# vocdoni/zk-franchise-proof-circuit

Measured on AMD Instinct MI355X. Metric: zkCensus proofs/sec (nLevels=160), higher is better.
Workload: dtype u256 (8 x u32 Montgomery, BN254 Fr/Fq)

## Files before the change

### include/zkcensus.h

```cpp
#ifndef ZKCENSUS_H
#define ZKCENSUS_H
#include <stddef.h>
#include <stdint.h>
#ifdef __cplusplus
extern "C" {
#endif

typedef struct zkc_ctx zkc_ctx;
typedef struct zkc_zkey zkc_zkey;

enum {
    ZKC_OK = 0,
    ZKC_ERR_GENERIC = 1,
    ZKC_ERR_SHORT_BUFFER = 2,
    ZKC_ERR_INVALID_WITNESS_LENGTH = 3,
    ZKC_ERR_BAD_ARG = 4,
    ZKC_ERR_FORMAT = 5,
    ZKC_ERR_HIP = 6,
    ZKC_ERR_WITNESS = 7
};
enum {
    ZKC_W_OK = 0, ZKC_W_ERR_WEIGHT = 1 , ZKC_W_ERR_SIK_ROOT = 2 ,
    ZKC_W_ERR_CENSUS_ROOT = 3 , ZKC_W_ERR_NULLIFIER = 4 , ZKC_W_ERR_LAST_SIBLING = 5 ,
    ZKC_W_ERR_INPUT_RANGE = 6 ,
// ... 81 lines not shown

int zkc_verify_batch(zkc_ctx* ctx, const uint8_t* vk, int nPublic, const uint8_t* pubs, const uint8_t* proofs, int N, const uint8_t* seed32);
const char* zkc_verify_last_error(void);

int zkc_proof_to_json(const uint8_t proof[256], const uint8_t* pub, int nPublic, char* proof_buf, unsigned long* proof_size,
                      char* public_buf, unsigned long* public_size);
int zkc_proof_from_json(const char* proof_json, const char* public_json, uint8_t proof[256], uint8_t* pub, int* nPublic);
int zkc_vkey_from_json(const char* vkey_json, uint8_t* vk, unsigned long* vk_size, int* nPublic);
int zkc_wtns_parse(const void* wtns_bytes, unsigned long size, const uint8_t** payload, uint32_t* nWitness);
unsigned long zkc_wtns_write(const void* payload, uint32_t nWitness, void* out, unsigned long out_size);

typedef struct zkc_msm zkc_msm;
int zkc_ntt_dev(zkc_ctx* ctx, const void* d_src, void* d_dst, int logn, int nvec, int inverse);
int zkc_g1_mul_batch_dev(zkc_ctx* ctx, const uint8_t base_std[64], const void* d_scalars, uint32_t n, void* d_out);
int zkc_msm_g1_load_dev(zkc_ctx* ctx, const void* d_bases_std, uint32_t n, zkc_msm** out);
int zkc_msm_g1_dev(zkc_msm* m, const void* d_scalars, uint8_t out[64]);
void zkc_msm_g1_free(zkc_msm* m);

int zkc_debug_stage(zkc_zkey* zk, const void* d_wtns, int stage, void* host_out);
unsigned long long zkc_debug_early_retries(void);
int zkc_msm_debug(zkc_zkey* zk, int which, const void* d_scalars, uint32_t count, void* host_out);
int zkc_debug_pairing_dev(zkc_ctx* ctx, const uint8_t* g1, const uint8_t* g2, const uint8_t* weights, int N, uint8_t product_out[384], uint8_t* folded_out,
                          int32_t* member_out, int* bad_out, const uint32_t* nodes, size_t count, uint8_t* node_out);

int zkc_poseidon_batch(zkc_ctx* ctx, int n_inputs, const void* inputs, size_t B, void* out);
int zkc_smt_build(zkc_ctx* ctx, const void* keys, const void* values, size_t n, int nLevels, uint8_t root[32], void* siblings, int32_t* depths);
int zkc_census_inputs(zkc_ctx* ctx, size_t n, int nLevels, const uint8_t election_id[64], const void* address, const void* password, const void* signature,
                      const void* available_weight, const void* vote_weight, const void* vote_hash, void* inputs_out, void* d_inputs_out, uint8_t* roots_out);

typedef struct zkc_tree zkc_tree;
enum {
    ZKC_TREE_OK = 0,
    ZKC_TREE_KEY_EXISTS = 1,
    ZKC_TREE_KEY_ABSENT = 2,
    ZKC_TREE_COLLISION = 3,
    ZKC_TREE_NOT_BELOW_R = 4,
    ZKC_TREE_NOT_IN_CENSUS = 5,
    ZKC_TREE_NOT_IN_SIK = 6,
    ZKC_TREE_SIK_MISMATCH = 7
};
int  zkc_tree_create(zkc_ctx* ctx, int nLevels, zkc_tree** out);
void zkc_tree_free(zkc_tree* tree);
int  zkc_tree_add(zkc_tree* tree, const void* keys, const void* values, size_t n, int32_t* status);
int  zkc_tree_update(zkc_tree* tree, const void* keys, const void* values, size_t n, int32_t* status);
int  zkc_tree_root(zkc_tree* tree, uint8_t root[32]);
int  zkc_tree_size(zkc_tree* tree, size_t* leaves);
// ... 38 lines not shown
```

### zk-franchise-proof-circuit_amd/__init__.py

```python
import ctypes
from . import _native
from ._native import ZkcError
from .inputs import INPUT_KEYS, flatten_inputs, R_MOD

__all__ = ['Context', 'ProvingKey', 'DevicePool', 'ProvingService', 'groth16', 'ZkcError', 'INPUT_KEYS', 'flatten_inputs', 'R_MOD']


class Context:

    def __init__(self, device=0):
        self._lib = _native.load()
        h = ctypes.c_void_p()
        rc = self._lib.zkc_ctx_create(int(device), ctypes.byref(h))
        if rc != 0:
            raise ZkcError(rc, (self._lib.zkc_last_error(None) or b'').decode())
        self._h = h
        self.device = device
        self._keys = []

    def close(self):
        if getattr(self, '_h', None):
            for k in list(self._keys):
                k.close()
            self._lib.zkc_ctx_destroy(self._h)
# ... 12 lines not shown

    @property
    def stream(self):
        return self._lib.zkc_ctx_stream(self._h)

    def n_wires(self, nLevels=160):
        return self._lib.zkc_circuit_n_wires(nLevels)

    def n_inputs(self, nLevels=160):
        return self._lib.zkc_circuit_n_inputs(nLevels)

    def witness(self, inputs, nLevels=160):
        flat = b''.join(x if isinstance(x, (bytes, bytearray)) else flatten_inputs(x, nLevels) for x in inputs)
        B = len(inputs)
        nw = self.n_wires(nLevels)
        out = ctypes.create_string_buffer(B * nw * 32)
        st = (ctypes.c_int32 * B)()
        self._check(self._lib.zkc_witness(self._h, nLevels, flat, B, out, st), allow=(7,))
        raw = out.raw
        return [raw[i * nw * 32:(i + 1) * nw * 32] for i in range(B)], list(st)

    def witness_dev(self, d_inputs_ptr, B, d_wtns_ptr, d_status_ptr, nLevels=160):
        self._check(self._lib.zkc_witness_dev(self._h, nLevels, d_inputs_ptr, B, d_wtns_ptr, d_status_ptr))


class ProvingKey:

    def __init__(self, ctx, zkey_bytes):
        self.ctx = ctx
        self._lib = ctx._lib
        h = ctypes.c_void_p()
        ctx._check(self._lib.zkc_zkey_load(ctx._h, zkey_bytes, len(zkey_bytes), ctypes.byref(h)))
        self._h = h
        ctx._keys.append(self)
        a, b, c = ctypes.c_uint32(), ctypes.c_uint32(), ctypes.c_uint32()
        self._lib.zkc_zkey_info(h, ctypes.byref(a), ctypes.byref(b), ctypes.byref(c))
        self.n_vars, self.n_public, self.domain_size = a.value, b.value, c.value
        ps, ln = ctypes.c_int(), ctypes.c_int()
        self._lib.zkc_zkey_pass_info(h, ctypes.byref(ps), ctypes.byref(ln))
        self.pass_size, self.lanes = ps.value, ln.value

    def close(self):
        if getattr(self, '_h', None):
            if getattr(self.ctx, '_h', None):
                self._lib.zkc_zkey_free(self._h)
            self._h = None
# ... 161 lines not shown
```

### zk-franchise-proof-circuit_amd/_native.py

```python
import ctypes
import os

_HERE = os.path.dirname(os.path.abspath(__file__))
LIB_PATH = os.environ.get('ZKCENSUS_LIB') or os.path.join(_HERE, 'libzkcensus.so')
_lib = None


class ZkcError(RuntimeError):
    def __init__(self, code, msg):
        super().__init__('libzkcensus error %d: %s' % (code, msg))
        self.code = code


def load():
    global _lib
    if _lib is not None:
        return _lib
    if not os.path.exists(LIB_PATH):
        raise ImportError('libzkcensus.so is not built (run `python -c "import __graft_entry__ as g; g.build()"`); '
                          'there is no CPU fallback for the product path')
    try:
        import torch
    except ImportError:
        pass
    L = ctypes.CDLL(LIB_PATH)
    vp, i32p = ctypes.c_void_p, ctypes.POINTER(ctypes.c_int32)
    L.zkc_ctx_create.argtypes = [ctypes.c_int, ctypes.POINTER(vp)]
    L.zkc_ctx_destroy.argtypes = [vp]
    L.zkc_last_error.argtypes = [vp]; L.zkc_last_error.restype = ctypes.c_char_p
    L.zkc_ctx_stream.argtypes = [vp]; L.zkc_ctx_stream.restype = vp
    L.zkc_witness.argtypes = [vp, ctypes.c_int, vp, ctypes.c_int, vp, i32p]
    L.zkc_witness_dev.argtypes = [vp, ctypes.c_int, vp, ctypes.c_int, vp, vp]
    u8p, u32p = ctypes.c_char_p, ctypes.POINTER(ctypes.c_uint32)
    L.zkc_zkey_load.argtypes = [vp, ctypes.c_char_p, ctypes.c_size_t, ctypes.POINTER(vp)]
    L.zkc_zkey_free.argtypes = [vp]; L.zkc_zkey_free.restype = None
    L.zkc_zkey_info.argtypes = [vp, u32p, u32p, u32p]
    L.zkc_zkey_pass_info.argtypes = [vp, ctypes.POINTER(ctypes.c_int), ctypes.POINTER(ctypes.c_int)]
    L.zkc_witness_status_text.argtypes = [ctypes.c_int, ctypes.c_int32]; L.zkc_witness_status_text.restype = ctypes.c_char_p
    L.zkc_prove.argtypes = [vp, ctypes.c_char_p, ctypes.c_uint32, u8p, u8p, ctypes.c_char_p, ctypes.c_char_p]
    L.zkc_prove_dev.argtypes = [vp, vp, ctypes.c_uint32, u8p, u8p, ctypes.c_char_p, ctypes.c_char_p]
    L.zkc_prove_batch_dev.argtypes = [vp, vp, ctypes.c_uint32, ctypes.c_int, ctypes.c_char_p, ctypes.c_char_p, ctypes.c_char_p]
    L.zkc_fullprove_batch_dev.argtypes = [vp, vp, ctypes.c_int, vp, vp, ctypes.c_char_p, ctypes.c_char_p, ctypes.c_char_p]
    L.zkc_debug_stage.argtypes = [vp, vp, ctypes.c_int, ctypes.c_char_p]
    L.zkc_debug_early_retries.argtypes = []; L.zkc_debug_early_retries.restype = ctypes.c_ulonglong
    L.zkc_msm_debug.argtypes = [vp, ctypes.c_int, vp, ctypes.c_uint32, ctypes.c_char_p]
    L.zkc_debug_pairing_dev.argtypes = [vp, ctypes.c_char_p, ctypes.c_char_p, ctypes.c_char_p, ctypes.c_int, ctypes.c_char_p, ctypes.c_char_p, i32p, ctypes.POINTER(ctypes.c_int),
                                        ctypes.POINTER(ctypes.c_uint32), ctypes.c_size_t, ctypes.c_char_p]
    ulp = ctypes.POINTER(ctypes.c_ulong)
    L.groth16_prover.argtypes = [ctypes.c_char_p, ctypes.c_ulong, ctypes.c_char_p, ctypes.c_ulong, ctypes.c_char_p, ulp, ctypes.c_char_p, ulp, ctypes.c_char_p, ctypes.c_ulong]
    L.zkc_verify.argtypes = [ctypes.c_char_p, ctypes.c_char_p, ctypes.c_char_p]
    L.zkc_verify_bin.argtypes = [ctypes.c_char_p, ctypes.c_int, ctypes.c_char_p, ctypes.c_char_p]
    L.zkc_verify_batch.argtypes = [vp, ctypes.c_char_p, ctypes.c_int, ctypes.c_char_p, ctypes.c_char_p, ctypes.c_int, ctypes.c_char_p]
    L.zkc_verify_batch_each.argtypes = [vp, ctypes.c_char_p, ctypes.c_int, ctypes.c_char_p, ctypes.c_char_p, ctypes.c_int, ctypes.c_char_p, i32p]
    L.zkc_verify_each_stats.argtypes = [vp, ctypes.POINTER(ctypes.c_uint64)]
    L.zkc_verify_last_error.restype = ctypes.c_char_p
    L.zkc_proof_to_json.argtypes = [ctypes.c_char_p, ctypes.c_char_p, ctypes.c_int, ctypes.c_char_p, ulp, ctypes.c_char_p, ulp]
    L.zkc_proof_from_json.argtypes = [ctypes.c_char_p, ctypes.c_char_p, ctypes.c_char_p, ctypes.c_char_p, ctypes.POINTER(ctypes.c_int)]
    L.zkc_vkey_from_json.argtypes = [ctypes.c_char_p, ctypes.c_char_p, ulp, ctypes.POINTER(ctypes.c_int)]
    L.zkc_wtns_parse.argtypes = [ctypes.c_char_p, ctypes.c_ulong, ctypes.POINTER(ctypes.c_void_p), ctypes.POINTER(ctypes.c_uint32)]
    L.zkc_wtns_write.argtypes = [ctypes.c_char_p, ctypes.c_uint32, ctypes.c_char_p, ctypes.c_ulong]; L.zkc_wtns_write.restype = ctypes.c_ulong
    L.zkc_poseidon_batch.argtypes = [vp, ctypes.c_int, ctypes.c_char_p, ctypes.c_size_t, ctypes.c_char_p]
    L.zkc_smt_build.argtypes = [vp, ctypes.c_char_p, ctypes.c_char_p, ctypes.c_size_t, ctypes.c_int, ctypes.c_char_p, ctypes.c_char_p, i32p]
    L.zkc_census_inputs.argtypes = [vp, ctypes.c_size_t, ctypes.c_int, ctypes.c_char_p, ctypes.c_char_p, ctypes.c_char_p, ctypes.c_char_p, ctypes.c_char_p, ctypes.c_char_p, ctypes.c_char_p, vp, vp, ctypes.c_char_p]
    sz = ctypes.c_size_t
    L.zkc_tree_create.argtypes = [vp, ctypes.c_int, ctypes.POINTER(vp)]
    L.zkc_tree_free.argtypes = [vp]; L.zkc_tree_free.restype = None
    L.zkc_tree_add.argtypes = [vp, ctypes.c_char_p, ctypes.c_char_p, sz, i32p]
    L.zkc_tree_update.argtypes = [vp, ctypes.c_char_p, ctypes.c_char_p, sz, i32p]
    L.zkc_tree_delete.argtypes = [vp, ctypes.c_char_p, sz, i32p]
    L.zkc_tree_refs.argtypes = [vp, ctypes.POINTER(sz)]
# ... 96 lines not shown
```

### zk-franchise-proof-circuit_amd/csrc/zkc_msm.hip

```cpp
#include <cstdio>
#include <cstddef>
#include <ctime>
#include <cstdlib>
#include <cstring>
#include <string.h>
#include <vector>
#include "zkc_prover.h"
#include "zkc_f29.h"
#include "zkc_f29_g1.h"
#include "zkc_f29_g2.h"
#include "zkc_point_ops.h"

namespace zkc {

template <class F> struct PointIO;
template <class PP> struct PointIO<Fp<PP>> {
    typedef Fp<PP> Fq;
    static __device__ __forceinline__ Affine<Fq> load(const Affine<Fq>* p) {
        const uint4* d = reinterpret_cast<const uint4*>(p); uint4 a = d[0], b = d[1], c = d[2], e = d[3];
        Affine<Fq> r;
        r.x.v[0] = a.x; r.x.v[1] = a.y; r.x.v[2] = a.z; r.x.v[3] = a.w; r.x.v[4] = b.x; r.x.v[5] = b.y; r.x.v[6] = b.z; r.x.v[7] = b.w;
        r.y.v[0] = c.x; r.y.v[1] = c.y; r.y.v[2] = c.z; r.y.v[3] = c.w; r.y.v[4] = e.x; r.y.v[5] = e.y; r.y.v[6] = e.z; r.y.v[7] = e.w;
        return r;
    }
// ... 497 lines not shown
    return fold_group_sums<Fq>(ctx, tbl, s, w, nw, sh, gs, ng, o, pt_mod, st);
}
int fold_group_sums_g1_ws(zkc_ctx* ctx, const G1Affine* tbl, const uint32_t* s, const uint32_t* w, uint32_t nw, const uint32_t* gs, uint32_t ng, G1XYZZ* d_tmp, G1XYZZ* d_out, G1XYZZ* h_out) {
    return fold_group_sums_ws<Fq>(ctx, tbl, s, w, nw, 0, gs, ng, d_tmp, d_out, h_out, 0u, ctx->stream);
}
int fold_group_sums_g2(zkc_ctx* ctx, const G2Affine* tbl, const uint32_t* s, const uint32_t* w, uint32_t nw, int32_t sh, const uint32_t* gs, uint32_t ng, G2XYZZ* o, uint32_t pt_mod, hipStream_t st) {
    return fold_group_sums<Fq2>(ctx, tbl, s, w, nw, sh, gs, ng, o, pt_mod, st);
}

static int msm_work_alloc_impl(zkc_ctx* ctx, MsmWork& w, size_t max_entries, size_t max_buckets, int max_jobs, bool g2) {
    w.max_entries = max_entries; w.max_jobs = max_jobs; w.max_buckets = max_buckets; w.xyzz_size = g2 ? sizeof(G2XYZZ) : sizeof(G1XYZZ);
    const size_t nb = max_buckets;
    w.max_segments = std::max<size_t>(max_entries / MSM_SEG + 1, (size_t)32 * 8192) + nb + 64;
    w.max_bins = (size_t)max_jobs << MSM_MAX_HBITS;
    ZKC_HIP_CHECK(ctx, hipMalloc((void**)&w.vals, max_entries * 4 + 16)); ZKC_HIP_CHECK(ctx, hipMalloc((void**)&w.vals2, max_entries * 4 + 16));
    ZKC_HIP_CHECK(ctx, hipMalloc((void**)&w.hist, w.max_bins * 4)); ZKC_HIP_CHECK(ctx, hipMalloc((void**)&w.bin_start, w.max_bins * 4));
    w.max_tilecnt = max_entries / 8 + ((size_t)max_jobs << MSM_MAX_HBITS);
    ZKC_HIP_CHECK(ctx, hipMalloc((void**)&w.tilecnt, w.max_tilecnt * 4));
    ZKC_HIP_CHECK(ctx, hipMalloc((void**)&w.off, (nb + 2) * 4)); ZKC_HIP_CHECK(ctx, hipMalloc((void**)&w.bcnt, (nb + 2) * 4)); ZKC_HIP_CHECK(ctx, hipMalloc((void**)&w.segcnt, (nb + 2) * 4));
    ZKC_HIP_CHECK(ctx, hipMalloc((void**)&w.segoff, (nb + 2) * 4)); ZKC_HIP_CHECK(ctx, hipMalloc((void**)&w.seg2bucket, w.max_segments * 4));
    ZKC_HIP_CHECK(ctx, hipMalloc((void**)&w.seglen, w.max_segments * 4)); ZKC_HIP_CHECK(ctx, hipMalloc((void**)&w.perm, w.max_segments * 4));
    w.max_lencnt = (size_t)(MSM_SEG + 1) * (w.max_segments / 256 + 2);
    ZKC_HIP_CHECK(ctx, hipMalloc((void**)&w.lencnt, w.max_lencnt * 4));
    ZKC_HIP_CHECK(ctx, hipMalloc((void**)&w.scan_blk, (std::max(nb + 2, w.max_lencnt) / 1024 + 2) * 4));
    ZKC_HIP_CHECK(ctx, hipMalloc((void**)&w.heavy, (MSM_MAX_HEAVY + 1) * 4));
    ZKC_HIP_CHECK(ctx, hipMalloc((void**)&w.d_jobs, sizeof(MsmJobList)));
    ZKC_HIP_CHECK(ctx, hipMalloc(&w.partial, w.max_segments * w.xyzz_size));
    const size_t max_vw = max_buckets / MSM_VW_MIN + (size_t)max_jobs;
    ZKC_HIP_CHECK(ctx, hipMalloc(&w.wres, 2 * max_vw * w.xyzz_size));
    ZKC_HIP_CHECK(ctx, hipMalloc((void**)&w.d_windows, max_vw * sizeof(MsmWindow))); w.max_windows = max_vw;
    w.max_tiles = max_entries / (8 * MSM_TILE_SCALARS) + (size_t)max_jobs + 1;
    ZKC_HIP_CHECK(ctx, hipMalloc((void**)&w.d_tilejob, w.max_tiles * 2));
    for (int s = 0; s < 2; s++) {
        ZKC_HIP_CHECK(ctx, hipHostMalloc((void**)&w.h_tilejob[s], w.max_tiles * 2));
        ZKC_HIP_CHECK(ctx, hipHostMalloc((void**)&w.h_jobs[s], sizeof(MsmJobList))); ZKC_HIP_CHECK(ctx, hipHostMalloc((void**)&w.h_windows[s], max_vw * sizeof(MsmWindow)));
        ZKC_HIP_CHECK(ctx, hipEventCreateWithFlags(&w.h_ev[s], hipEventDisableTiming));
    }
    ZKC_HIP_CHECK(ctx, hipMalloc(&w.results, 2 * (size_t)max_jobs * w.xyzz_size));
    ZKC_HIP_CHECK(ctx, hipHostMalloc(&w.h_results, (size_t)max_jobs * w.xyzz_size));
    return ZKC_OK;
}
int msm_work_alloc(zkc_ctx* ctx, MsmWork& w, size_t max_entries, size_t max_buckets, int max_jobs, bool g2) {
    const int rc = msm_work_alloc_impl(ctx, w, max_entries, max_buckets, max_jobs, g2);
    if (rc != ZKC_OK) msm_work_free(w);
    return rc;
}
void msm_work_free(MsmWork& w) {
// ... 142 lines not shown
```

### zk-franchise-proof-circuit_amd/csrc/zkc_msm_sort.hip

```cpp
#include "zkc_prover.h"
#include <algorithm>

namespace zkc {

struct TileState { uint32_t s[MSM_TILE_SCALARS / MSM_TILE][8]; uint32_t pt[MSM_TILE_SCALARS / MSM_TILE]; uint32_t carry[MSM_TILE_SCALARS / MSM_TILE]; bool live[MSM_TILE_SCALARS / MSM_TILE]; };
__device__ __forceinline__ void msm_tile_load(TileState& t, const MsmJob& job, uint32_t i0) {
#pragma unroll
    for (int k = 0; k < MSM_TILE_SCALARS / MSM_TILE; k++) {
        const uint32_t i = i0 + k * MSM_TILE;
        t.live[k] = i < job.count; t.pt[k] = 0; t.carry[k] = 0;
#pragma unroll
        for (int q = 0; q < 8; q++) t.s[k][q] = 0;
        if (t.live[k]) {
            const uint32_t wire = job.vmap ? job.vmap[i] : i;
            const uint4* sp = reinterpret_cast<const uint4*>(job.scalars + 8 * (size_t)wire); const uint4 a = sp[0], b = sp[1];
            t.s[k][0] = a.x; t.s[k][1] = a.y; t.s[k][2] = a.z; t.s[k][3] = a.w; t.s[k][4] = b.x; t.s[k][5] = b.y; t.s[k][6] = b.z; t.s[k][7] = b.w;
            t.pt[k] = (uint32_t)((int32_t)wire - job.pt_shift);
        }
    }
}
__device__ __forceinline__ uint32_t msm_tile_digit(TileState& t, int k, uint32_t w, uint32_t c, uint32_t& neg) {
    const uint32_t half = 1u << (c - 1), mask = (1u << c) - 1;
    const uint32_t bit = w * c, li = bit >> 5, sh = bit & 31;
    uint32_t lo = 0, hi = 0;
// ... 248 lines not shown
    if (valid && wave > 0) rank += wcnt[(wave - 1) * LEN_KEYS + key];
    return rank;
}
__global__ void __launch_bounds__(256)
zkc_msm_lenhist(const uint32_t* __restrict__ seglen, const uint32_t* __restrict__ segoff, uint32_t nbuckets, uint32_t* __restrict__ lencnt, uint32_t max_segments) {
    __shared__ uint32_t wcnt[4 * LEN_KEYS];
    uint32_t nseg = segoff[nbuckets]; if (nseg > max_segments) nseg = max_segments;
    const uint32_t s = blockIdx.x * 256 + threadIdx.x;
    const bool valid = s < nseg;
    const uint32_t key = valid ? (uint32_t)MSM_SEG - seglen[s] : ~0u;
    (void)stable_rank_256(key, valid, wcnt);
    for (uint32_t k = threadIdx.x; k < LEN_KEYS; k += 256) lencnt[(size_t)k * gridDim.x + blockIdx.x] = wcnt[3 * LEN_KEYS + k];
}
__global__ void __launch_bounds__(256)
zkc_msm_lenscatter(const uint32_t* __restrict__ seglen, const uint32_t* __restrict__ segoff, uint32_t nbuckets, const uint32_t* __restrict__ lencnt,
                   uint32_t* __restrict__ perm, uint32_t max_segments) {
    __shared__ uint32_t wcnt[4 * LEN_KEYS];
    uint32_t nseg = segoff[nbuckets]; if (nseg > max_segments) nseg = max_segments;
    const uint32_t s = blockIdx.x * 256 + threadIdx.x;
    const bool valid = s < nseg;
    const uint32_t key = valid ? (uint32_t)MSM_SEG - seglen[s] : ~0u;
    const uint32_t rank = stable_rank_256(key, valid, wcnt);
    if (valid) perm[lencnt[(size_t)key * gridDim.x + blockIdx.x] + rank] = s;
}

#define ZKC_SORT_LAUNCH_CHECK(name) do { hipError_t _e = hipGetLastError(); if (_e != hipSuccess) return zkc_fail(ctx, ZKC_ERR_HIP, std::string(name ": ") + hipGetErrorString(_e)); } while (0)

int msm_bucket_entries(zkc_ctx* ctx, MsmWork& w, const MsmJobList& jl, hipStream_t st, unsigned long long* d_entry_counter) {
    if (jl.total_bins > w.max_bins) return zkc_fail(ctx, ZKC_ERR_BAD_ARG, "msm_bucket_entries: too many level-1 bins for the work space");
    const MsmJobList* dj = (const MsmJobList*)w.d_jobs;
    if (jl.total_tilecnt > w.max_tilecnt) return zkc_fail(ctx, ZKC_ERR_BAD_ARG, "msm_bucket_entries: too many (bin, tile) counters for the work space");
    hipLaunchKernelGGL(zkc_msm_count, dim3(jl.total_tiles), dim3(MSM_TILE), 0, st, dj, (const uint16_t*)w.d_tilejob, w.tilecnt);
    ZKC_SORT_LAUNCH_CHECK("zkc_msm_count");
    hipLaunchKernelGGL(zkc_msm_binscan, dim3(jl.njobs), dim3(256), 0, st, dj, w.tilecnt, w.hist, w.bin_start, d_entry_counter);
    ZKC_SORT_LAUNCH_CHECK("zkc_msm_binscan");
    hipLaunchKernelGGL(zkc_msm_split, dim3(jl.total_tiles), dim3(MSM_TILE), 0, st, dj, (const uint16_t*)w.d_tilejob, w.tilecnt, w.vals);
    ZKC_SORT_LAUNCH_CHECK("zkc_msm_split");
    uint64_t biggest_bin = 0;
    for (int j = 0; j < jl.njobs; j++) biggest_bin = std::max<uint64_t>(biggest_bin, ((uint64_t)jl.job[j].count * jl.job[j].nw) >> jl.job[j].hbits);
    if (biggest_bin > 8192) hipLaunchKernelGGL(HIP_KERNEL_NAME(zkc_msm_bucket<true>), dim3(jl.total_bins), dim3(256), 0, st, dj, w.hist, w.bin_start, w.vals, w.vals2, w.off, w.bcnt);
    else hipLaunchKernelGGL(HIP_KERNEL_NAME(zkc_msm_bucket<false>), dim3(jl.total_bins), dim3(256), 0, st, dj, w.hist, w.bin_start, w.vals, w.vals2, w.off, w.bcnt);
    ZKC_SORT_LAUNCH_CHECK("zkc_msm_bucket");
    return ZKC_OK;
}

static int device_scan(zkc_ctx* ctx, const uint32_t* in, uint32_t* out, uint32_t* blk, uint32_t n, hipStream_t st) {
    const uint32_t nblk = (n + SCAN_PER_BLOCK - 1) / SCAN_PER_BLOCK;
    hipLaunchKernelGGL(zkc_scan_local, dim3(nblk), dim3(256), 0, st, in, out, blk, n);
    hipLaunchKernelGGL(zkc_scan_blocks, dim3(1), dim3(256), 0, st, blk, nblk);
    hipLaunchKernelGGL(zkc_scan_fix, dim3((n + 255) / 256), dim3(256), 0, st, out, blk, n);
    ZKC_SORT_LAUNCH_CHECK("zkc_scan");
    return ZKC_OK;
}
int msm_build_segments(zkc_ctx* ctx, MsmWork& w, const MsmJobList& jl, uint32_t seg, size_t seg_bound, hipStream_t st) {
    const uint32_t nb = jl.total_buckets;
    if (seg > (uint32_t)MSM_SEG) return zkc_fail(ctx, ZKC_ERR_BAD_ARG, "msm_build_segments: segment length");
    ZKC_HIP_CHECK(ctx, hipMemsetAsync(w.heavy + MSM_MAX_HEAVY, 0, 4, st));
    hipLaunchKernelGGL(zkc_msm_segcount, dim3((nb + 1 + 255) / 256), dim3(256), 0, st, w.bcnt, nb, w.segcnt, w.heavy, w.heavy + MSM_MAX_HEAVY, seg);
    ZKC_SORT_LAUNCH_CHECK("zkc_msm_segcount");
    int rc = device_scan(ctx, w.segcnt, w.segoff, w.scan_blk, nb + 1, st); if (rc) return rc;
    const bool sort_by_len = seg > (uint32_t)MSM_SEG_MIN * 2;
    hipLaunchKernelGGL(zkc_msm_seg2bucket, dim3((nb + 255) / 256), dim3(256), 0, st, w.bcnt, w.segoff, nb, w.seg2bucket, w.seglen, (uint32_t)w.max_segments, sort_by_len ? nullptr : w.perm);
    ZKC_SORT_LAUNCH_CHECK("zkc_msm_seg2bucket");
    if (!sort_by_len) return ZKC_OK;
    const uint32_t nwg = (uint32_t)((seg_bound + 255) / 256), nlen = LEN_KEYS * nwg;
    if ((size_t)nlen > w.max_lencnt) return zkc_fail(ctx, ZKC_ERR_BAD_ARG, "msm_build_segments: too many segments for the work space");
    hipLaunchKernelGGL(zkc_msm_lenhist, dim3(nwg), dim3(256), 0, st, w.seglen, w.segoff, nb, w.lencnt, (uint32_t)w.max_segments);
    ZKC_SORT_LAUNCH_CHECK("zkc_msm_lenhist");
    rc = device_scan(ctx, w.lencnt, w.lencnt, w.scan_blk, nlen, st); if (rc) return rc;
    hipLaunchKernelGGL(zkc_msm_lenscatter, dim3(nwg), dim3(256), 0, st, w.seglen, w.segoff, nb, w.lencnt, w.perm, (uint32_t)w.max_segments);
    ZKC_SORT_LAUNCH_CHECK("zkc_msm_lenscatter");
    return ZKC_OK;
}

}
```

### zk-franchise-proof-circuit_amd/csrc/zkc_prover.h

```cpp
#pragma once
#include <cstring>
#include "zkc_internal.h"
#include "zkc_curve.h"
#include "zkc_abc_rows.h"
#include "zkc_top_fold.h"
#include "zkc_pass_plan.h"
#include <array>

namespace zkc {
constexpr int MSM_C_BIG = 17, MSM_C_SMALL = 12;
inline long long first_unreduced_wire(const void* w, size_t count) {
    const uint8_t* p = (const uint8_t*)w;
    for (size_t i = 0; i < count; i++) {
        uint32_t t[8]; memcpy(t, p + 32 * i, 32);
        if (t[7] >= FrParams::p[7] && !fp_std_lt_p<FrParams>(t)) return (long long)i;
    }
    return -1;
}
inline std::string unreduced_wire_msg(long long wire) { return "Witness value at wire " + std::to_string(wire) + " is not below the field order r"; }
inline int msm_c_for(size_t W) { return W < 12000 ? 12 : W < 22000 ? 13 : W < 90000 ? 15 : W < 180000 ? 16 : 17; }
constexpr int MSM_VW_MIN = 64, MSM_MAX_VW_PER_JOB = 64;
constexpr int MSM_MAX_VW_G1 = 256;
constexpr int MSM_SEG_MIN = 16;
#ifndef ZKC_MSM_SEG
// ... 81 lines not shown
        if (hbits_big != 0xffu && hbits_small != 0xffu) {
            const uint32_t lim = nbig << hbits_big;
            return bin < lim ? bin >> hbits_big : nbig + ((bin - lim) >> hbits_small);
        }
        uint32_t lo = 0, hi = (uint32_t)njobs - 1;
        while (lo < hi) { const uint32_t mid = (lo + hi + 1) >> 1; if (job[mid].bin0 <= bin) lo = mid; else hi = mid - 1; }
        return lo;
    }
    ZKC_HD void decode(uint32_t id, uint32_t& d, uint32_t& j) const {
        const uint32_t lim = hb * nbig;
        if (id < lim) { j = id / hb; d = id - j * hb; }
        else { const uint32_t t = id - lim, q = t / hs; j = nbig + q; d = t - q * hs; }
    }
};
struct MsmWindow { uint32_t bucket0, out, per; };

struct MsmWork {
    uint32_t *vals = nullptr, *vals2 = nullptr;
    uint32_t *hist = nullptr, *bin_start = nullptr;
    uint32_t *tilecnt = nullptr; size_t max_tilecnt = 0;
    uint32_t *off = nullptr, *bcnt = nullptr;
    uint32_t *segcnt = nullptr, *segoff = nullptr, *seg2bucket = nullptr, *heavy = nullptr;
    uint32_t *seglen = nullptr, *perm = nullptr;
    uint32_t *scan_blk = nullptr, *lencnt = nullptr; size_t max_lencnt = 0;
    void *partial = nullptr;
    void *wres = nullptr;
    void *results = nullptr;
    void *h_results = nullptr;
    MsmJobList* d_jobs = nullptr;
    MsmWindow* d_windows = nullptr; size_t max_buckets = 0, max_bins = 0, max_windows = 0;
    uint16_t* d_tilejob = nullptr; uint16_t* h_tilejob[2] = {nullptr, nullptr}; size_t max_tiles = 0;
    MsmJobList* h_jobs[2] = {nullptr, nullptr}; MsmWindow* h_windows[2] = {nullptr, nullptr}; hipEvent_t h_ev[2] = {nullptr, nullptr}; int h_next = 0;
    size_t max_entries = 0, max_segments = 0; int max_jobs = 0; size_t xyzz_size = 0;
};
}

struct zkc_lane {
    hipStream_t st = nullptr, st2 = nullptr, fin = nullptr;
    hipStream_t red = nullptr; hipEvent_t ev_red = nullptr;
    zkc::Fr *d_abc = nullptr, *d_t = nullptr; uint32_t* d_p = nullptr;
    void* d_fin = nullptr;
    uint32_t* d_bs = nullptr;
    zkc::MsmWork w1, w2;
    size_t cap_abc = 0, cap_p = 0, cap_fin = 0, cap_bs = 0, bytes = 0; bool made = false;
    hipEvent_t ev_msm = nullptr, ev_msm2 = nullptr, ev_sorted = nullptr, ev_ntt = nullptr, ev_mv = nullptr, ev_acc = nullptr, ev_fin[2] = {nullptr, nullptr}; int npass = 0;
};

// ... 114 lines not shown
```

### zk-franchise-proof-circuit_amd/csrc/zkc_switches.h

```cpp
#pragma once
#include <climits>
#include <cstdlib>
#include <optional>

namespace zkc { namespace sw {

enum Kind { SET, OFF_IF_ZERO, ON_IF_ONE, NUMBER, NUMBER_LONG, NUMBER_U64, TEXT };
enum When { PROCESS, LIVE };
constexpr long long ANY = LLONG_MIN;

#define ZKC_SWITCHES(X)                                                                                                                                                   \
                                                                                                                                            \
    X(ZKC_DEVICE,               TEXT,        ANY, ANY,   LIVE,    "service creation: the GPUs of the default proving service: \"2\", \"0,1,2,3\", \"all\"; unset: every visible device") \
    X(ZKC_INFLIGHT,             NUMBER,      1,   128,   LIVE,    "key load: proofs per pipeline pass (census key 64, any other 96, fewer for a large circuit); at most MSM_MAX_JOBS / 4") \
    X(ZKC_LANES,                NUMBER,      1,   4,     LIVE,    "key load: pipeline lanes the passes of a batch call rotate over (census key MAX_LANES = 4, any other 1)")      \
    X(ZKC_DEEP_TABLES,          NUMBER,      ANY, ANY,   LIVE,    "key load: 0 leaves out the second section tables that passes of deep voters take, 2 builds them for a census key of any size (default 1)") \
    X(ZKC_G2_LONE_TABLE,        OFF_IF_ZERO, ANY, ANY,   LIVE,    "key load: =0 skips the 8-bit-window G2 table of the lone-proof path")                                          \
    X(ZKC_BLIND_TREE,           OFF_IF_ZERO, ANY, ANY,   LIVE,    "key load: =0 gives a key whose passes of one or two proofs take the general blinding kernels")                 \
    X(ZKC_SERVICE_WORKERS,      NUMBER,      1,   4,     LIVE,    "service creation: workers (= lanes of a service key) per GPU (4); at most MAX_LANES")                          \
    X(ZKC_SERVICE_PASS,         NUMBER,      1,   128,   LIVE,    "service creation: proofs per pass of a service key (64); at most MSM_MAX_JOBS / 4")                            \
    X(ZKC_SERVICE_KEYS,         NUMBER,      1,   64,    LIVE,    "service creation: keys kept resident per GPU (4)")                                                             \
    X(ZKC_SERVICE_MAX_BATCH,    NUMBER,      1,   4096,  LIVE,    "service creation: requests one worker takes per call (256)")                                                   \
    X(ZKC_SERVICE_MIN_BATCH,    NUMBER,      1,   ANY,   LIVE,    "service creation: requests a collecting worker waits for before it goes (16)")                                 \
    X(ZKC_SERVICE_SPILL,        NUMBER,      1,   ANY,   LIVE,    "service creation: queue length at which a cold GPU is brought up (32)")                                        \
    X(ZKC_SERVICE_BUSY_WAIT_US, NUMBER,      0,   ANY,   LIVE,    "service creation: microseconds a collecting worker waits for more requests (300)")                             \
    X(ZKC_SERVICE_RESERVE,      OFF_IF_ZERO, ANY, ANY,   PROCESS, "=0: a service key load does not reserve a full pass of work space on every lane; the lanes grow on demand")    \
    X(ZKC_DEVICE_BLOCKING_SYNC, ON_IF_ONE,   ANY, ANY,   LIVE,    "context creation: =1 asks HIP for blocking waits on the device (hipDeviceScheduleBlockingSync)")               \
    X(ZKC_SPIN_WAIT,            SET,         ANY, ANY,   PROCESS, "set (any value, 0 included): host waits use hipEventSynchronize instead of polling with short sleeps")         \
    X(ZKC_VERIFY_BATCH_GPU,     NUMBER,      ANY, ANY,   LIVE,    "per verify call: 0 keeps the Miller loops of zkc_verify_batch on the host, positive forces the GPU, negative or unset: GPU from 128 proofs") \
    X(ZKC_NO_SHA_NI,            SET,         ANY, ANY,   PROCESS, "set (any value, 0 included): portable SHA-256 instead of the CPU's SHA extensions")                            \
                                                                                                                              \
    X(ZKC_NO_FOLD,              SET,         ANY, ANY,   LIVE,    "key load: set (any value, 0 included): no constant folding of the voter-independent witness part for this key") \
    X(ZKC_SERIAL_STREAMS,       SET,         ANY, ANY,   LIVE,    "key load: set (any value, 0 included): every stage of this key's passes on the context's one stream (isolated stage times)") \
    X(ZKC_C_SECTIONS,           NUMBER,      8,   17,    LIVE,    "key load: window bits of the witness sections (census key 12, any other by its wire count); at most MSM_C_BIG") \
    X(ZKC_C_H,                  NUMBER,      8,   17,    LIVE,    "key load: window bits of the H section (census key 17, any other by its domain size); at most MSM_C_BIG")      \
    X(ZKC_C_DEEP,               NUMBER,      13,  17,    LIVE,    "key load: window bits of the second section tables (by the wire count); at most MSM_C_BIG")                    \
    X(ZKC_DEEP_WIRES,           NUMBER_LONG, ANY, ANY,   PROCESS, "live wires per section and proof from which a pass takes the second section tables (16000)")                   \
    X(ZKC_WITNESS_GROUP,        NUMBER,      1,   ANY,   PROCESS, "passes whose voters share one witness launch in a batch call (8)")                                             \
    X(ZKC_VW_BIG,               NUMBER,      ANY, ANY,   PROCESS, "buckets per reduction wave of the H jobs in passes of more than four proofs (0 or unset: 4096, 1024 below 32 proofs)") \
    X(ZKC_VW_SMALL,             NUMBER,      ANY, ANY,   PROCESS, "the same for the witness sections (0 or unset: 2048, 256 below 32 proofs)")                                    \
    X(ZKC_VW_G2,                NUMBER,      ANY, ANY,   PROCESS, "the same for the G2 jobs of passes of 32 proofs and more (0 or unset: as the witness sections)")              \
    X(ZKC_G2_ACC,               NUMBER,      ANY, ANY,   PROCESS, "form of the G2 accumulation: 0 registers hold the next row, 1 / 2 LDS-DMA prefetch at one / two waves per SIMD (0)") \
    X(ZKC_G2_BUCKET_WAVE,       OFF_IF_ZERO, ANY, ANY,   PROCESS, "=0: small G2 passes keep lane-per-segment accumulation instead of half a wave per bucket")                     \
    X(ZKC_G2_LATE,              SET,         ANY, ANY,   PROCESS, "set (any value, 0 included): the G2 MSM of a pass starts after the G1 sort instead of with the pass")          \
    X(ZKC_G2_ACC_HOLD,          SET,         ANY, ANY,   PROCESS, "set (any value, 0 included): the G2 accumulation always waits for the G1 stream to leave its transforms")      \
    X(ZKC_G2_ACC_EARLY,         SET,         ANY, ANY,   PROCESS, "set (any value, 0 included): the G2 accumulation never waits for them (ZKC_G2_ACC_HOLD wins)")                 \
    X(ZKC_ACC_CHAIN,            OFF_IF_ZERO, ANY, ANY,   PROCESS, "=0: the G1 accumulations of a context's lanes are not chained one behind the other")                           \
    X(ZKC_REDUCE_STREAM,        ON_IF_ONE,   ANY, ANY,   PROCESS, "=1: the bucket reduction of a full pass runs on a stream of its own (the lanes then get that stream)")         \
    X(ZKC_MATVEC_UNITS,         OFF_IF_ZERO, ANY, ANY,   PROCESS, "=0: buildABC multiplies by its +-1 coefficients instead of adding the wire")                                   \
    X(ZKC_ABC_FOLD,             OFF_IF_ZERO, ANY, ANY,   PROCESS, "=0: buildABC of a folded pass computes every row instead of copying the voter-independent ones from the template") \
    X(ZKC_TOP_FOLD,             NUMBER,      0,   12,    LIVE,    "key load: census tree levels below the root whose MSM terms are summed once per subtree instead of per voter (8; 0: off)") \
    X(ZKC_MATVEC_INLINE,        SET,        ANY, ANY,   PROCESS, "set (any value, 0 included): buildABC of the next pass is not prefetched on the blinding stream")              \
    X(ZKC_MV_PREFETCH_AT_NTT,   ON_IF_ONE,   ANY, ANY,   PROCESS, "=1: that prefetch starts beside the pass' bucketing instead of beside its accumulation")                       \
    X(ZKC_EARLY_LAYOUT,         OFF_IF_ZERO, ANY, ANY,   PROCESS, "=0: one-pass calls of more than two voters wait for their fold flags instead of reading the depths off the inputs") \
    X(ZKC_NOFOLD_LISTS,         OFF_IF_ZERO, ANY, ANY,   PROCESS, "=0: unfolded passes keep the wires whose bases are at infinity")                                               \
    X(ZKC_NTT_SEPARATE,         SET,         ANY, ANY,   PROCESS, "set (any value, 0 included): two self-contained transforms instead of the fused pair")                         \
    X(ZKC_NTT_RADIX,            NUMBER,      ANY, ANY,   PROCESS, "below 4: the head transform kernel runs one stage at a time instead of two (4)")                               \
    X(ZKC_FINALIZE_WAVES,       SET,         ANY, ANY,   PROCESS, "set (any value, 0 included): the one-wave-per-task blinding kernel for every pass")                            \
    X(ZKC_VERIFY_CHUNK,         NUMBER,      2,   16384, LIVE,    "per verify call: pairs per round of Miller-loop kernels (16384)")                                              \
    X(ZKC_SMT_WAVE_MAX,         NUMBER_U64,  ANY, ANY,   LIVE,    "per check call: census proof batches up to this size take the wave-per-proof form (64; 0: never)")            \
    X(ZKC_TRACE_HOST,           SET,         ANY, ANY,   PROCESS, "set (any value, 0 included): prints where the enqueueing thread spends its time, per pass")                    \
    X(ZKC_VERIFY_TRACE,         SET,         ANY, ANY,   LIVE,    "per verify call: set (any value, 0 included): prints the stage times of zkc_verify_batch")                     \
    X(ZKC_DEBUG_SYNC,           SET,         ANY, ANY,   PROCESS, "set (any value, 0 included): synchronises after and logs every MSM launch; read when the library is loaded")   \
                                                                                                                                                \
    X(ZKC_TEST_FAIL_ALLOC,      NUMBER,      ANY, ANY,   LIVE,    "lane growth: the work-space allocation for this many proofs in flight or more fails")                          \
    X(ZKC_TEST_TOP_SLOTS,       NUMBER,      1,   16384, LIVE,    "key load: slots per tree of the top-of-tree table instead of 8 x 2^K (1: every subtree lands on one slot)")    \
    X(ZKC_TEST_FAIL_KEY_LOADS,  NUMBER,      ANY, ANY,   LIVE,    "service key load: fails as out of memory while the device holds this many keys or more")

enum Id {
// ... 43 lines not shown
```

Baseline: 3407.

## Build MSM segment lists with three fused kernels instead of eleven commands

Replaces the memset plus ten-launch segment-building sequence (segment count, scans, length histogram, length scatter) with three kernels: a per-block count that also builds the per-length histogram, a single scan kernel that handles block totals and per-key offsets including the max_segments cut, and an emit kernel that writes offsets, seg2bucket, heavy buckets and the length-sorted permutation. The goal is to cut per-pass launch overhead and global round trips in MSM bucketing. The new path is on by default behind a switch, and the scan scratch buffer is enlarged. A debug entry point is added to compare the fused and unfused outputs. The catch is more complex boundary handling around truncation at max_segments.

```diff
diff --git a/include/zkcensus.h b/include/zkcensus.h
--- a/include/zkcensus.h
+++ b/include/zkcensus.h
@@ -127,6 +127,9 @@
 int zkc_msm_debug(zkc_zkey* zk, int which, const void* d_scalars, uint32_t count, void* host_out);
 int zkc_debug_pairing_dev(zkc_ctx* ctx, const uint8_t* g1, const uint8_t* g2, const uint8_t* weights, int N, uint8_t product_out[384], uint8_t* folded_out,
                           int32_t* member_out, int* bad_out, const uint32_t* nodes, size_t count, uint8_t* node_out);
+#define ZKC_DEBUG_SEGMENTS_CANARY 0x5e9c0de5u
+int zkc_debug_build_segments(zkc_ctx* ctx, const uint32_t* bcnt, uint32_t nb, uint32_t seg, uint32_t max_segments, int fused, uint32_t* segcnt, uint32_t* segoff,
+                             uint32_t* seg2bucket, uint32_t* perm, uint32_t* heavy, uint32_t* nheavy);
 
 int zkc_poseidon_batch(zkc_ctx* ctx, int n_inputs, const void* inputs, size_t B, void* out);
 int zkc_smt_build(zkc_ctx* ctx, const void* keys, const void* values, size_t n, int nLevels, uint8_t root[32], void* siblings, int32_t* depths);
diff --git a/zk-franchise-proof-circuit_amd/__init__.py b/zk-franchise-proof-circuit_amd/__init__.py
--- a/zk-franchise-proof-circuit_amd/__init__.py
+++ b/zk-franchise-proof-circuit_amd/__init__.py
@@ -58,6 +58,20 @@
 
     def witness_dev(self, d_inputs_ptr, B, d_wtns_ptr, d_status_ptr, nLevels=160):
         self._check(self._lib.zkc_witness_dev(self._h, nLevels, d_inputs_ptr, B, d_wtns_ptr, d_status_ptr))
+
+    SEGMENTS_CANARY = 0x5e9c0de5
+
+    def debug_build_segments(self, bcnt, seg, max_segments, fused=True):
+        import numpy as np
+        bcnt = np.ascontiguousarray(bcnt, dtype=np.uint32); nb = int(bcnt.size)
+        u32p = ctypes.POINTER(ctypes.c_uint32); ptr = lambda a: a.ctypes.data_as(u32p)
+        segcnt, segoff = np.zeros(nb + 2, np.uint32), np.zeros(nb + 2, np.uint32)
+        seg2bucket, perm = np.zeros(int(max_segments) + 1, np.uint32), np.zeros(int(max_segments) + 1, np.uint32)
+        heavy, nheavy = np.zeros(max(nb, 1), np.uint32), ctypes.c_uint32()
+        self._check(self._lib.zkc_debug_build_segments(self._h, ptr(bcnt), nb, int(seg), int(max_segments), int(bool(fused)), ptr(segcnt), ptr(segoff), ptr(seg2bucket),
+                                                       ptr(perm), ptr(heavy), ctypes.byref(nheavy)))
+        return {'segcnt': segcnt[:nb + 1], 'segoff': segoff[:nb + 1], 'seg2bucket': seg2bucket[:-1], 'perm': perm[:-1], 'heavy': heavy[:min(nheavy.value, nb)],
+                'nheavy': nheavy.value, 'canary': np.array([segcnt[-1], segoff[-1], seg2bucket[-1], perm[-1]], np.uint32)}
 
 
 class ProvingKey:
diff --git a/zk-franchise-proof-circuit_amd/_native.py b/zk-franchise-proof-circuit_amd/_native.py
--- a/zk-franchise-proof-circuit_amd/_native.py
+++ b/zk-franchise-proof-circuit_amd/_native.py
@@ -46,6 +46,7 @@
     L.zkc_msm_debug.argtypes = [vp, ctypes.c_int, vp, ctypes.c_uint32, ctypes.c_char_p]
     L.zkc_debug_pairing_dev.argtypes = [vp, ctypes.c_char_p, ctypes.c_char_p, ctypes.c_char_p, ctypes.c_int, ctypes.c_char_p, ctypes.c_char_p, i32p, ctypes.POINTER(ctypes.c_int),
                                         ctypes.POINTER(ctypes.c_uint32), ctypes.c_size_t, ctypes.c_char_p]
+    L.zkc_debug_build_segments.argtypes = [vp, u32p, ctypes.c_uint32, ctypes.c_uint32, ctypes.c_uint32, ctypes.c_int, u32p, u32p, u32p, u32p, u32p, u32p]
     ulp = ctypes.POINTER(ctypes.c_ulong)
     L.groth16_prover.argtypes = [ctypes.c_char_p, ctypes.c_ulong, ctypes.c_char_p, ctypes.c_ulong, ctypes.c_char_p, ulp, ctypes.c_char_p, ulp, ctypes.c_char_p, ctypes.c_ulong]
     L.zkc_verify.argtypes = [ctypes.c_char_p, ctypes.c_char_p, ctypes.c_char_p]
diff --git a/zk-franchise-proof-circuit_amd/csrc/zkc_msm.hip b/zk-franchise-proof-circuit_amd/csrc/zkc_msm.hip
--- a/zk-franchise-proof-circuit_amd/csrc/zkc_msm.hip
+++ b/zk-franchise-proof-circuit_amd/csrc/zkc_msm.hip
@@ -543,7 +543,8 @@
     ZKC_HIP_CHECK(ctx, hipMalloc((void**)&w.seglen, w.max_segments * 4)); ZKC_HIP_CHECK(ctx, hipMalloc((void**)&w.perm, w.max_segments * 4));
     w.max_lencnt = (size_t)(MSM_SEG + 1) * (w.max_segments / 256 + 2);
     ZKC_HIP_CHECK(ctx, hipMalloc((void**)&w.lencnt, w.max_lencnt * 4));
-    ZKC_HIP_CHECK(ctx, hipMalloc((void**)&w.scan_blk, (std::max(nb + 2, w.max_lencnt) / 1024 + 2) * 4));
+    w.max_scan_blk = std::max(nb + 2, w.max_lencnt) / 1024 + 2 + 2 * ((nb + 1) / 1024 + 1) + 1;
+    ZKC_HIP_CHECK(ctx, hipMalloc((void**)&w.scan_blk, w.max_scan_blk * 4));
     ZKC_HIP_CHECK(ctx, hipMalloc((void**)&w.heavy, (MSM_MAX_HEAVY + 1) * 4));
     ZKC_HIP_CHECK(ctx, hipMalloc((void**)&w.d_jobs, sizeof(MsmJobList)));
     ZKC_HIP_CHECK(ctx, hipMalloc(&w.partial, w.max_segments * w.xyzz_size));
diff --git a/zk-franchise-proof-circuit_amd/csrc/zkc_msm_sort.hip b/zk-franchise-proof-circuit_amd/csrc/zkc_msm_sort.hip
--- a/zk-franchise-proof-circuit_amd/csrc/zkc_msm_sort.hip
+++ b/zk-franchise-proof-circuit_amd/csrc/zkc_msm_sort.hip
@@ -294,6 +294,123 @@
     const uint32_t key = valid ? (uint32_t)MSM_SEG - seglen[s] : ~0u;
     const uint32_t rank = stable_rank_256(key, valid, wcnt);
     if (valid) perm[lencnt[(size_t)key * gridDim.x + blockIdx.x] + rank] = s;
+}
+
+constexpr uint32_t SEG_BLOCK = 1024;
+static_assert(LEN_KEYS <= 256, "a workgroup scans the per-key totals in one round");
+__global__ void __launch_bounds__(256)
+zkc_msm_seg_count(const uint32_t* __restrict__ bcnt, uint32_t nbuckets, uint32_t seg, uint32_t* __restrict__ segcnt, uint32_t* __restrict__ segoff, uint32_t* __restrict__ blk,
+                  uint32_t* __restrict__ heavy_count, uint32_t* __restrict__ lencnt) {
+    __shared__ uint32_t sh[256];
+    __shared__ uint32_t hist[LEN_KEYS];
+    if (lencnt) for (uint32_t k = threadIdx.x; k < LEN_KEYS; k += 256) hist[k] = 0;
+    const uint32_t b0 = blockIdx.x * SEG_BLOCK + threadIdx.x * 4;
+    uint32_t L[4], c[4], sum = 0;
+#pragma unroll
+    for (int k = 0; k < 4; k++) { L[k] = b0 + k < nbuckets ? bcnt[b0 + k] : 0; c[k] = (L[k] + seg - 1) / seg; sum += c[k]; }
+    uint32_t total; uint32_t run = block_excl_scan_256(sum, sh, total);
+#pragma unroll
+    for (int k = 0; k < 4; k++) { if (b0 + k <= nbuckets) { segcnt[b0 + k] = c[k]; segoff[b0 + k] = run; } run += c[k]; }
+    if (threadIdx.x == 0) { blk[blockIdx.x] = total; if (blockIdx.x == 0) *heavy_count = 0; }
+    if (!lencnt) return;
+#pragma unroll
+    for (int k = 0; k < 4; k++) if (c[k]) {
+        const uint32_t q = L[k] / c[k], r = L[k] - q * c[k];
+        if (r) atomicAdd(&hist[(uint32_t)MSM_SEG - (q + 1)], r);
+        atomicAdd(&hist[(uint32_t)MSM_SEG - q], c[k] - r);
+    }
+    __syncthreads();
+    for (uint32_t k = threadIdx.x; k < LEN_KEYS; k += 256) lencnt[(size_t)k * gridDim.x + blockIdx.x] = hist[k];
+}
+template <class V, class P>
+__device__ __forceinline__ uint32_t wg_excl_scan(uint32_t n, uint32_t* sh, V value, P put) {
+    uint32_t carry = 0;
+    for (uint32_t base = 0; base < n; base += 1024) {
+        uint32_t v[4], sum = 0;
+#pragma unroll
+        for (int k = 0; k < 4; k++) { const uint32_t i = base + threadIdx.x * 4 + k; v[k] = i < n ? value(i) : 0; sum += v[k]; }
+        uint32_t total; uint32_t run = carry + block_excl_scan_256(sum, sh, total);
+#pragma unroll
+        for (int k = 0; k < 4; k++) { const uint32_t i = base + threadIdx.x * 4 + k; if (i < n) put(i, run, v[k]); run += v[k]; }
+        carry += total;
+    }
+    return carry;
+}
+__global__ void __launch_bounds__(256)
+zkc_msm_seg_scan(const uint32_t* __restrict__ blk, uint32_t nblk, uint32_t* __restrict__ blkbase, uint32_t* __restrict__ lencnt, uint32_t max_segments,
+                 const uint32_t* __restrict__ bcnt, const uint32_t* __restrict__ segcnt, const uint32_t* __restrict__ segoff, uint32_t nbuckets) {
+    __shared__ uint32_t sh[256];
+    __shared__ uint32_t cut[4];
+    const bool owner = blockIdx.x == gridDim.x - 1;
+    if (threadIdx.x == 0) { cut[0] = nblk; cut[1] = ~0u; cut[2] = 0; cut[3] = 0; }
+    __syncthreads();
+    const uint32_t total = wg_excl_scan(nblk, sh, [&](uint32_t i) { return blk[i]; }, [&](uint32_t i, uint32_t run, uint32_t v) {
+        if (owner) blkbase[i] = run;
+        if (run >= max_segments) atomicMin(&cut[0], i); else if (run + v > max_segments) { cut[1] = i; cut[2] = run; }
+    });
+    if (owner && threadIdx.x == 0) blkbase[nblk] = total;
+    if (!lencnt || owner) return;
+    __syncthreads();
+    const uint32_t key = blockIdx.x, dead = cut[0], across = cut[1];
+    if (across != ~0u) {
+        uint32_t cnt = 0;
+        for (uint32_t i = threadIdx.x; i < SEG_BLOCK; i += 256) {
+            const uint32_t b = across * SEG_BLOCK + i;
+            if (b >= nbuckets) break;
+            const uint32_t k = segcnt[b], s0 = cut[2] + segoff[b], L = bcnt[b];
+            if (!k || s0 >= max_segments) continue;
+            if (k <= max_segments - s0) { const uint32_t q = L / k, r = L - q * k; cnt += (r && (uint32_t)MSM_SEG - (q + 1) == key ? r : 0) + ((uint32_t)MSM_SEG - q == key ? k - r : 0); }
+            else for (uint32_t j = 0; j < max_segments - s0; j++) { uint32_t lo, hi; msm_seg_range_s(L, k, j, lo, hi); cnt += (uint32_t)MSM_SEG - (hi - lo) == key; }
+        }
+        if (cnt) atomicAdd(&cut[3], cnt);
+        __syncthreads();
+    }
+    const uint32_t recount = cut[3];
+    uint32_t* row = lencnt + (size_t)key * nblk;
+    const uint32_t ktotal = wg_excl_scan(nblk, sh, [&](uint32_t i) { return i >= dead ? 0u : i == across ? recount : row[i]; }, [&](uint32_t i, uint32_t run, uint32_t) { row[i] = run; });
+    if (threadIdx.x == 0) lencnt[(size_t)LEN_KEYS * nblk + key] = ktotal;
+}
+__global__ void __launch_bounds__(256)
+zkc_msm_seg_emit(const uint32_t* __restrict__ bcnt, uint32_t nbuckets, const uint32_t* __restrict__ blkbase, uint32_t* __restrict__ segoff, uint32_t* __restrict__ seg2bucket,
+                 uint32_t* __restrict__ perm, const uint32_t* __restrict__ lencnt, uint32_t* __restrict__ heavy, uint32_t* __restrict__ heavy_count, uint32_t max_segments) {
+    __shared__ uint32_t loff[SEG_BLOCK + 1], lcnt[SEG_BLOCK];
+    __shared__ uint32_t wcnt[4 * LEN_KEYS], kbase[LEN_KEYS], sh[256];
+    const uint32_t nblk = gridDim.x, base = blkbase[blockIdx.x], nseg_blk = blkbase[blockIdx.x + 1] - base, b0 = blockIdx.x * SEG_BLOCK;
+#pragma unroll
+    for (int k = 0; k < 4; k++) {
+        const uint32_t i = threadIdx.x * 4 + k, b = b0 + i;
+        uint32_t o = nseg_blk;
+        if (b <= nbuckets) { o = segoff[b]; segoff[b] = base + o; }
+        loff[i] = o; lcnt[i] = b < nbuckets ? bcnt[b] : 0;
+    }
+    if (threadIdx.x == 0) loff[SEG_BLOCK] = nseg_blk;
+    __syncthreads();
+#pragma unroll
+    for (int k = 0; k < 4; k++) {
+        const uint32_t i = threadIdx.x * 4 + k;
+        if (loff[i + 1] - loff[i] > (uint32_t)MSM_MERGE_T) { const uint32_t h = atomicAdd(heavy_count, 1u); if (h < (uint32_t)MSM_MAX_HEAVY) heavy[h] = b0 + i; }
+    }
+    if (lencnt) {
+        const uint32_t v = threadIdx.x < LEN_KEYS ? lencnt[(size_t)LEN_KEYS * nblk + threadIdx.x] : 0;
+        uint32_t all; const uint32_t ahead = block_excl_scan_256(v, sh, all);
+        if (threadIdx.x < LEN_KEYS) kbase[threadIdx.x] = ahead + lencnt[(size_t)threadIdx.x * nblk + blockIdx.x];
+        __syncthreads();
+    }
+    const uint32_t listed = base >= max_segments ? 0 : nseg_blk < max_segments - base ? nseg_blk : max_segments - base;
+    for (uint32_t c0 = 0; c0 < listed; c0 += 256) {
+        const uint32_t ls = c0 + threadIdx.x, s = base + ls; const bool valid = ls < listed;
+        uint32_t lo = 0, hi = SEG_BLOCK - 1;
+        if (valid) while (lo < hi) { const uint32_t mid = (lo + hi + 1) >> 1; if (loff[mid] <= ls) lo = mid; else hi = mid - 1; }
+        if (valid) seg2bucket[s] = b0 + lo;
+        if (!lencnt) { if (valid) perm[s] = s; continue; }
+        uint32_t key = ~0u;
+        if (valid) { uint32_t e0, e1; msm_seg_range_s(lcnt[lo], loff[lo + 1] - loff[lo], ls - loff[lo], e0, e1); key = (uint32_t)MSM_SEG - (e1 - e0); }
+        const uint32_t rank = stable_rank_256(key, valid, wcnt);
+        if (valid) { const uint32_t p = kbase[key] + rank; if (p < max_segments) perm[p] = s; }
+        __syncthreads();
+        if (threadIdx.x < LEN_KEYS) kbase[threadIdx.x] += wcnt[3 * LEN_KEYS + threadIdx.x];
+        __syncthreads();
+    }
 }
 
 #define ZKC_SORT_LAUNCH_CHECK(name) do { hipError_t _e = hipGetLastError(); if (_e != hipSuccess) return zkc_fail(ctx, ZKC_ERR_HIP, std::string(name ": ") + hipGetErrorString(_e)); } while (0)
@@ -324,9 +441,22 @@
     ZKC_SORT_LAUNCH_CHECK("zkc_scan");
     return ZKC_OK;
 }
-int msm_build_segments(zkc_ctx* ctx, MsmWork& w, const MsmJobList& jl, uint32_t seg, size_t seg_bound, hipStream_t st) {
-    const uint32_t nb = jl.total_buckets;
-    if (seg > (uint32_t)MSM_SEG) return zkc_fail(ctx, ZKC_ERR_BAD_ARG, "msm_build_segments: segment length");
+static int build_segments_fused(zkc_ctx* ctx, MsmWork& w, uint32_t nb, uint32_t seg, hipStream_t st) {
+    const uint32_t nblk = (nb + 1 + SEG_BLOCK - 1) / SEG_BLOCK;
+    const bool sort_by_len = seg > (uint32_t)MSM_SEG_MIN * 2;
+    if ((size_t)LEN_KEYS * (nblk + 1) > w.max_lencnt || 2 * (size_t)nblk + 1 > w.max_scan_blk) return zkc_fail(ctx, ZKC_ERR_BAD_ARG, "msm_build_segments: too many buckets for the work space");
+    uint32_t* const blkbase = w.scan_blk + nblk; uint32_t* const lencnt = sort_by_len ? w.lencnt : nullptr;
+    hipLaunchKernelGGL(zkc_msm_seg_count, dim3(nblk), dim3(256), 0, st, w.bcnt, nb, seg, w.segcnt, w.segoff, w.scan_blk, w.heavy + MSM_MAX_HEAVY, lencnt);
+    ZKC_SORT_LAUNCH_CHECK("zkc_msm_seg_count");
+    hipLaunchKernelGGL(zkc_msm_seg_scan, dim3(sort_by_len ? LEN_KEYS + 1 : 1), dim3(256), 0, st, w.scan_blk, nblk, blkbase, lencnt, (uint32_t)w.max_segments, w.bcnt, w.segcnt, w.segoff, nb);
+    ZKC_SORT_LAUNCH_CHECK("zkc_msm_seg_scan");
+    hipLaunchKernelGGL(zkc_msm_seg_emit, dim3(nblk), dim3(256), 0, st, w.bcnt, nb, blkbase, w.segoff, w.seg2bucket, w.perm, lencnt, w.heavy, w.heavy + MSM_MAX_HEAVY, (uint32_t)w.max_segments);
+    ZKC_SORT_LAUNCH_CHECK("zkc_msm_seg_emit");
+    return ZKC_OK;
+}
+static int build_segments(zkc_ctx* ctx, MsmWork& w, uint32_t nb, uint32_t seg, size_t seg_bound, hipStream_t st, bool fused) {
+    if (seg < 1 || seg > (uint32_t)MSM_SEG) return zkc_fail(ctx, ZKC_ERR_BAD_ARG, "msm_build_segments: segment length");
+    if (fused) return build_segments_fused(ctx, w, nb, seg, st);
     ZKC_HIP_CHECK(ctx, hipMemsetAsync(w.heavy + MSM_MAX_HEAVY, 0, 4, st));
     hipLaunchKernelGGL(zkc_msm_segcount, dim3((nb + 1 + 255) / 256), dim3(256), 0, st, w.bcnt, nb, w.segcnt, w.heavy, w.heavy + MSM_MAX_HEAVY, seg);
     ZKC_SORT_LAUNCH_CHECK("zkc_msm_segcount");
@@ -344,5 +474,50 @@
     ZKC_SORT_LAUNCH_CHECK("zkc_msm_lenscatter");
     return ZKC_OK;
 }
-
-}
+int msm_build_segments(zkc_ctx* ctx, MsmWork& w, const MsmJobList& jl, uint32_t seg, size_t seg_bound, hipStream_t st) {
+    return build_segments(ctx, w, jl.total_buckets, seg, seg_bound, st, sw::on<sw::ZKC_SEG_FUSED>());
+}
+
+}
+
+extern "C" int zkc_debug_build_segments(zkc_ctx* ctx, const uint32_t* bcnt, uint32_t nb, uint32_t seg, uint32_t max_segments, int fused, uint32_t* segcnt, uint32_t* segoff,
+                                        uint32_t* seg2bucket, uint32_t* perm, uint32_t* heavy, uint32_t* nheavy) {
+    using namespace zkc;
+    if (!ctx) return ZKC_ERR_BAD_ARG;
+    if (!bcnt || !segcnt || !segoff || !seg2bucket || !perm || !heavy || !nheavy || nb < 1 || nb > (1u << 26) || seg < 1 || seg > (uint32_t)MSM_SEG || max_segments < 1 ||
+        max_segments > (1u << 27)) return zkc_fail(ctx, ZKC_ERR_BAD_ARG, "zkc_debug_build_segments: bad argument");
+    uint64_t total = 0;
+    for (uint32_t b = 0; b < nb; b++) total += bcnt[b];
+    if (total >= (1ull << 31)) return zkc_fail(ctx, ZKC_ERR_BAD_ARG, "zkc_debug_build_segments: too many entries");
+    ZKC_LOCK(ctx);
+    ZKC_HIP_CHECK(ctx, hipSetDevice(ctx->device));
+    const hipStream_t st = ctx->stream;
+    const size_t seg_bound = (size_t)(total / seg) + nb, nblk = ((size_t)nb + 1 + SEG_BLOCK - 1) / SEG_BLOCK;
+    MsmWork w;
+    w.max_segments = max_segments; w.max_buckets = nb;
+    w.max_lencnt = (size_t)LEN_KEYS * std::max((seg_bound + 255) / 256 + 1, nblk + 1);
+    w.max_scan_blk = std::max((size_t)nb + 2, w.max_lencnt) / SCAN_PER_BLOCK + 2 + 2 * nblk + 1;
+    struct Out { uint32_t** dev; size_t words; uint32_t* host; };
+    const Out outs[4] = {{&w.segcnt, (size_t)nb + 1, segcnt}, {&w.segoff, (size_t)nb + 1, segoff}, {&w.seg2bucket, max_segments, seg2bucket}, {&w.perm, max_segments, perm}};
+    DevBuf d_out[4], d_bcnt, d_seglen, d_lencnt, d_blk, d_heavy; int rc;
+    const uint32_t canary = ZKC_DEBUG_SEGMENTS_CANARY;
+    for (int k = 0; k < 4; k++) {
+        if ((rc = d_out[k].alloc(ctx, (outs[k].words + 1) * 4))) return rc;
+        *outs[k].dev = d_out[k].as<uint32_t>();
+        ZKC_HIP_CHECK(ctx, hipMemsetAsync(d_out[k].p, 0xff, outs[k].words * 4, st));
+        ZKC_HIP_CHECK(ctx, hipMemcpyAsync(d_out[k].as<uint32_t>() + outs[k].words, &canary, 4, hipMemcpyHostToDevice, st));
+    }
+    if ((rc = d_bcnt.alloc(ctx, ((size_t)nb + 2) * 4)) || (rc = d_seglen.alloc(ctx, (size_t)max_segments * 4)) || (rc = d_lencnt.alloc(ctx, w.max_lencnt * 4)) ||
+        (rc = d_blk.alloc(ctx, w.max_scan_blk * 4)) || (rc = d_heavy.alloc(ctx, ((size_t)MSM_MAX_HEAVY + 1) * 4))) return rc;
+    w.bcnt = d_bcnt.as<uint32_t>(); w.seglen = d_seglen.as<uint32_t>(); w.lencnt = d_lencnt.as<uint32_t>(); w.scan_blk = d_blk.as<uint32_t>(); w.heavy = d_heavy.as<uint32_t>();
+    ZKC_HIP_CHECK(ctx, hipMemsetAsync(d_bcnt.p, 0, ((size_t)nb + 2) * 4, st));
+    ZKC_HIP_CHECK(ctx, hipMemcpyAsync(w.bcnt, bcnt, (size_t)nb * 4, hipMemcpyHostToDevice, st));
+    ZKC_HIP_CHECK(ctx, hipMemsetAsync(w.heavy + MSM_MAX_HEAVY, 0xff, 4, st));
+    if ((rc = build_segments(ctx, w, nb, seg, seg_bound, st, fused != 0))) return rc;
+    ZKC_HIP_CHECK(ctx, hipStreamSynchronize(st));
+    for (int k = 0; k < 4; k++) ZKC_HIP_CHECK(ctx, hipMemcpy(outs[k].host, d_out[k].p, (outs[k].words + 1) * 4, hipMemcpyDeviceToHost));
+    ZKC_HIP_CHECK(ctx, hipMemcpy(nheavy, w.heavy + MSM_MAX_HEAVY, 4, hipMemcpyDeviceToHost));
+    const uint32_t listed = std::min<uint32_t>(std::min<uint32_t>(*nheavy, (uint32_t)MSM_MAX_HEAVY), nb);
+    if (listed) ZKC_HIP_CHECK(ctx, hipMemcpy(heavy, w.heavy, (size_t)listed * 4, hipMemcpyDeviceToHost));
+    return ZKC_OK;
+}
diff --git a/zk-franchise-proof-circuit_amd/csrc/zkc_prover.h b/zk-franchise-proof-circuit_amd/csrc/zkc_prover.h
--- a/zk-franchise-proof-circuit_amd/csrc/zkc_prover.h
+++ b/zk-franchise-proof-circuit_amd/csrc/zkc_prover.h
@@ -127,7 +127,7 @@
     uint32_t *off = nullptr, *bcnt = nullptr;
     uint32_t *segcnt = nullptr, *segoff = nullptr, *seg2bucket = nullptr, *heavy = nullptr;
     uint32_t *seglen = nullptr, *perm = nullptr;
-    uint32_t *scan_blk = nullptr, *lencnt = nullptr; size_t max_lencnt = 0;
+    uint32_t *scan_blk = nullptr, *lencnt = nullptr; size_t max_lencnt = 0, max_scan_blk = 0;
     void *partial = nullptr;
     void *wres = nullptr;
     void *results = nullptr;
diff --git a/zk-franchise-proof-circuit_amd/csrc/zkc_switches.h b/zk-franchise-proof-circuit_amd/csrc/zkc_switches.h
--- a/zk-franchise-proof-circuit_amd/csrc/zkc_switches.h
+++ b/zk-franchise-proof-circuit_amd/csrc/zkc_switches.h
@@ -45,6 +45,7 @@
     X(ZKC_G2_LATE,              SET,         ANY, ANY,   PROCESS, "set (any value, 0 included): the G2 MSM of a pass starts after the G1 sort instead of with the pass")          \
     X(ZKC_G2_ACC_HOLD,          SET,         ANY, ANY,   PROCESS, "set (any value, 0 included): the G2 accumulation always waits for the G1 stream to leave its transforms")      \
     X(ZKC_G2_ACC_EARLY,         SET,         ANY, ANY,   PROCESS, "set (any value, 0 included): the G2 accumulation never waits for them (ZKC_G2_ACC_HOLD wins)")                 \
+    X(ZKC_SEG_FUSED,            OFF_IF_ZERO, ANY, ANY,   PROCESS, "=0: the segment lists of a pass are built by eleven commands per side (memset, ten launches) instead of three launches") \
     X(ZKC_ACC_CHAIN,            OFF_IF_ZERO, ANY, ANY,   PROCESS, "=0: the G1 accumulations of a context's lanes are not chained one behind the other")                           \
     X(ZKC_REDUCE_STREAM,        ON_IF_ONE,   ANY, ANY,   PROCESS, "=1: the bucket reduction of a full pass runs on a stream of its own (the lanes then get that stream)")         \
     X(ZKC_MATVEC_UNITS,         OFF_IF_ZERO, ANY, ANY,   PROCESS, "=0: buildABC multiplies by its +-1 coefficients instead of adding the wire")                                   \
```

Result: no change. 3432 (median of 6 runs) (+0.7%).
